# Siyou-Li/u2Tokenizer

Measured on NVIDIA H100. Metric: ct_volumes_per_sec, higher is better.
Workload: dtype bf16

## Files before the change

include/u2b200.h:

```cpp
#ifndef U2B200_H_
#define U2B200_H_

#include <stdint.h>

#if defined(__GNUC__)
#define U2_API __attribute__((visibility("default")))
#else
#define U2_API
#endif

#ifdef __cplusplus
extern "C" {
#endif

#define U2_OK 0
#define U2_ERR_ARG (-1)
#define U2_ERR_CUDA (-2)
#define U2_ERR_UNSUPPORTED (-3)

#define U2_DT_BF16 0
#define U2_DT_F32 1

#define U2_ACT_NONE 0
#define U2_ACT_GELU 1
// ... 97 lines not shown
} u2_rope_desc;
U2_API int u2_rope_bf16(void* x, const u2_rope_desc* desc, void* stream);

U2_API int u2_decode_attention_bf16(const void* q, const void* k_cache, const void* v_cache, void* out,
                                    int32_t B, int32_t Hq, int32_t Hkv, int32_t dh, int32_t Tmax, int32_t T,
                                    const int32_t* T_dev, int64_t ldq, int64_t ldo, float scale, int32_t T_per_seq,
                                    const int32_t* kv_src, int64_t ld_kv_src, void* stream);
U2_API int u2_decode_attention_window_bf16(const void* q, const void* k_cache, const void* v_cache, void* out,
                                           int32_t B, int32_t Hq, int32_t Hkv, int32_t dh, int32_t Tmax, int32_t T,
                                           const int32_t* T_dev, int64_t ldq, int64_t ldo, float scale,
                                           int32_t T_per_seq, const int32_t* kv_src, int64_t ld_kv_src,
                                           int32_t window, void* stream);

typedef struct u2_gemv_desc {
  int32_t B, N, K;
  int64_t ldx, ldw, ldy, ldr;
  int32_t y_dtype;
  const void* residual;
  const float* norm_gamma;
  float norm_eps;
  int32_t silu_pair;
} u2_gemv_desc;
U2_API int u2_gemv_bf16(const void* x, const void* w, void* y, const u2_gemv_desc* desc, void* stream);
U2_API int u2_argmax_f32(const float* logits, int64_t* out, uint64_t* scratch, int32_t B, int32_t V, int64_t ld,
                         void* stream);

#define U2_DLIN_STREAMK128 0
#define U2_DLIN_TILES64 1
typedef struct u2_dlinear_desc {
  int32_t B, N, K;
  int64_t ldx, ldw, ldy, ldr, ldxg;
  int32_t y_dtype;
  float* ws;
  int32_t* counters;
  const float* ssq_in;
  float eps;
  const void* residual;
  int32_t silu_pair;
  const float* gamma_next;
  void* xg;
  float* ssq_out;
  float* ssq_zero;
  int32_t pdl;
  void* dbg;
  int64_t ws_elems;
  const int32_t* dep_flags;
  int32_t dep_shift;
  int32_t* out_flags;
  int32_t sched;
} u2_dlinear_desc;
U2_API int u2_dlinear_bf16(const void* x, const void* w, void* y, const u2_dlinear_desc* desc, void* stream);
U2_API int64_t u2_dlinear_ws_elems(int32_t N, int32_t K);
typedef struct u2_dlinear_next {
  int32_t pre_stages;
  int32_t lookahead_units;
  int32_t n;
  const void* w[2];
  int32_t N[2], K[2];
  int64_t ldw[2];
  int32_t units[2];
} u2_dlinear_next;
U2_API int u2_dlinear_multi_bf16(const void* const* x, const void* const* w, void* const* y,
                                 const u2_dlinear_desc* descs, int32_t n_ops, uint32_t* gridbar,
                                 const int32_t* step_dev, int32_t pdl, const u2_dlinear_next* next, void* stream);
U2_API int u2_decode_embed_bf16(const int64_t* ids, const void* table, const float* gamma, void* x, void* xg,
                                float* ssq, float* ssq_zero, int32_t* step_counter, int32_t B, int32_t E,
                                int64_t vocab, void* stream);

typedef struct u2_fused_decode_desc {
  int32_t B, Hq, Hkv, dh, Tmax, pos;
  const int32_t* pos_dev;
  int64_t ldq, ldo;
  const float* q_norm_w;
  const float* k_norm_w;
  float eps;
  const float* inv_freq;
  float scale;
  int32_t kv_splits;
  int32_t pdl;
  int32_t pos_per_seq;
  const int32_t* kv_src;
  int64_t ld_kv_src;
  int32_t window;
} u2_fused_decode_desc;
U2_API int u2_decode_attention_fused_bf16(const void* qkv, void* k_cache, void* v_cache, void* out,
                                          const u2_fused_decode_desc* desc, void* stream);

U2_API int u2_topk_rows_f32(const float* scores, int64_t* out_idx, int32_t rows, int32_t T, int32_t K, int64_t ld,
                            int64_t idx_offset_per_row, void* stream);

typedef struct u2_fa_desc {
  int32_t B, H, Sq, Sk, dh;
  float scale;
  int64_t q_sb, q_ss, q_sh;
  int64_t k_sb, k_ss, k_sh;
  int64_t v_sb, v_ss, v_sh;
  int64_t out_sb, out_ss;
  float* lse;
} u2_fa_desc;
U2_API int u2_flash_attention_d64_bf16(const void* q, const void* k, const void* v, void* out, const u2_fa_desc* desc,
                                       void* stream);

U2_API int u2_sample_f32(const float* logits, int64_t* out, int32_t B, int32_t V, int64_t ld, float temperature,
                         int32_t top_k, float top_p, uint64_t seed, const int32_t* step_dev, int32_t step,
                         void* stream);

typedef struct u2_sample_params {
  float temperature;
  int32_t top_k;
  float top_p;
  int32_t reserved;
  uint64_t seed;
} u2_sample_params;
U2_API int u2_sample_dev_f32(const float* logits, int64_t* out, int32_t B, int32_t V, int64_t ld,
                             const u2_sample_params* params_dev, const int32_t* step_dev, int32_t step, void* stream);

#define U2_LP_MAX_EOS 8
#define U2_LP_MAX_BAD_WORDS 256
#define U2_LP_MAX_BAD_TOKENS 2048
typedef struct u2_logits_proc_params {
  float penalty;
  float inv_penalty;
  int32_t ngram;
  int32_t min_new;
  int32_t n_eos;
  int32_t n_bad;
  int32_t eos[U2_LP_MAX_EOS];
  int32_t bad_off[U2_LP_MAX_BAD_WORDS + 1];
  int32_t bad_tok[U2_LP_MAX_BAD_TOKENS];
} u2_logits_proc_params;
U2_API int u2_logits_process_f32(float* logits, int32_t B, int32_t V, int64_t ld, const int64_t* ids, int32_t* hist,
                                 int64_t ld_hist, int32_t hist_cap, const u2_logits_proc_params* params_dev,
                                 const int32_t* step_dev, int32_t step, void* stream);

#define U2_BEAM_MAX_BEAMS 16
#define U2_BEAM_MAX_EOS 8
#define U2_BEAM_MAX_KEEP 144
typedef struct u2_beam_params {
  double length_penalty;
  int32_t num_beams;
  int32_t beams_to_keep;
  int32_t early_stopping;
  int32_t max_new_tokens;
  int32_t n_eos;
  int32_t reserved;
  int32_t eos[U2_BEAM_MAX_EOS];
} u2_beam_params;
typedef struct u2_beam_step_desc {
  const u2_beam_params* params;
  int32_t prompts, V;
  const float* cand_val;
  const int32_t* cand_tok;
  float* running;
  float* fin_score;
  int32_t* fin_info;
  int32_t* flags;
  int64_t* ids;
  int32_t* rec;
  int64_t ld_rec;
  int32_t rec_rows;
  int32_t* kv_src;
  int64_t ld_kv_src;
  const int32_t* pos_dev;
  int32_t* hist;
  int64_t ld_hist;
  int32_t hist_cap;
// ... 50 lines not shown
```

u2tokenizer_b200/_lib.py:

```python
from __future__ import annotations

import ctypes as C
from pathlib import Path

_LIB_PATH = Path(__file__).resolve().parent / "libu2b200.so"
_lib = None


class GemmDesc(C.Structure):
    _fields_ = [
        ("M", C.c_int32), ("N", C.c_int32), ("K", C.c_int32),
        ("zi", C.c_int32), ("zo", C.c_int32), ("b_zi_div", C.c_int32),
        ("lda", C.c_int64), ("a_stride_zi", C.c_int64), ("a_stride_zo", C.c_int64),
        ("ldb", C.c_int64), ("b_stride_zi", C.c_int64), ("b_stride_zo", C.c_int64),
        ("ldc", C.c_int64), ("c_stride_zi", C.c_int64), ("c_stride_zo", C.c_int64),
        ("c_dtype", C.c_int32), ("alpha", C.c_float),
        ("bias", C.c_void_p),
        ("act", C.c_int32),
        ("residual", C.c_void_p),
        ("ldr", C.c_int64),
        ("res_row_mod", C.c_int32),
        ("row_div", C.c_int32), ("row_stride", C.c_int32), ("row_off", C.c_int32),
        ("block_n", C.c_int32),
        ("a_mn", C.c_int32), ("b_mn", C.c_int32),
# ... 1 lines not shown
        ("rowvec", C.c_void_p),
        ("rv_stride_zi", C.c_int64), ("rv_stride_zo", C.c_int64),
        ("mul", C.c_void_p),
    ]


class SoftmaxDesc(C.Structure):
    _fields_ = [
        ("in_s0", C.c_int64), ("in_s1", C.c_int64), ("in_s2", C.c_int64),
        ("out_s0", C.c_int64), ("out_s1", C.c_int64), ("out_s2", C.c_int64),
        ("n0", C.c_int32), ("H", C.c_int32), ("S", C.c_int32), ("n", C.c_int32),
        ("scale", C.c_float),
        ("rel_bias", C.c_void_p),
        ("rel_max", C.c_int32),
        ("causal", C.c_int32), ("causal_off", C.c_int32),
        ("zero_pad_to", C.c_int32),
        ("window", C.c_int32),
    ]


class RopeDesc(C.Structure):
    _fields_ = [
        ("rows", C.c_int64), ("ld", C.c_int64),
        ("dh", C.c_int32), ("n_q_heads", C.c_int32), ("n_k_heads", C.c_int32), ("n_v_heads", C.c_int32),
        ("q_norm_w", C.c_void_p), ("k_norm_w", C.c_void_p),
        ("eps", C.c_float),
        ("inv_freq", C.c_void_p),
        ("pos0", C.c_int32), ("pos_div", C.c_int32), ("pos_mod", C.c_int32),
        ("pos0_dev", C.c_void_p),
        ("k_cache", C.c_void_p), ("v_cache", C.c_void_p),
        ("Tmax", C.c_int32), ("rows_per_batch", C.c_int32),
        ("pos0_per_batch", C.c_int32),
    ]


class GemvDesc(C.Structure):
    _fields_ = [
        ("B", C.c_int32), ("N", C.c_int32), ("K", C.c_int32),
        ("ldx", C.c_int64), ("ldw", C.c_int64), ("ldy", C.c_int64), ("ldr", C.c_int64),
        ("y_dtype", C.c_int32),
        ("residual", C.c_void_p),
        ("norm_gamma", C.c_void_p),
        ("norm_eps", C.c_float),
        ("silu_pair", C.c_int32),
    ]


class DlinearDesc(C.Structure):
    _fields_ = [
        ("B", C.c_int32), ("N", C.c_int32), ("K", C.c_int32),
        ("ldx", C.c_int64), ("ldw", C.c_int64), ("ldy", C.c_int64), ("ldr", C.c_int64), ("ldxg", C.c_int64),
        ("y_dtype", C.c_int32),
        ("ws", C.c_void_p), ("counters", C.c_void_p),
        ("ssq_in", C.c_void_p),
        ("eps", C.c_float),
        ("residual", C.c_void_p),
        ("silu_pair", C.c_int32),
        ("gamma_next", C.c_void_p),
        ("xg", C.c_void_p),
        ("ssq_out", C.c_void_p),
        ("ssq_zero", C.c_void_p),
        ("pdl", C.c_int32),
        ("dbg", C.c_void_p),
        ("ws_elems", C.c_int64),
        ("dep_flags", C.c_void_p), ("dep_shift", C.c_int32), ("out_flags", C.c_void_p),
        ("sched", C.c_int32),
    ]


class FusedDecodeDesc(C.Structure):
    _fields_ = [
        ("B", C.c_int32), ("Hq", C.c_int32), ("Hkv", C.c_int32), ("dh", C.c_int32), ("Tmax", C.c_int32),
        ("pos", C.c_int32),
        ("pos_dev", C.c_void_p),
        ("ldq", C.c_int64), ("ldo", C.c_int64),
        ("q_norm_w", C.c_void_p), ("k_norm_w", C.c_void_p),
        ("eps", C.c_float),
        ("inv_freq", C.c_void_p),
        ("scale", C.c_float),
        ("kv_splits", C.c_int32), ("pdl", C.c_int32),
        ("pos_per_seq", C.c_int32),
        ("kv_src", C.c_void_p), ("ld_kv_src", C.c_int64),
        ("window", C.c_int32),
    ]


class DlinearNext(C.Structure):
    _fields_ = [
        ("pre_stages", C.c_int32), ("lookahead_units", C.c_int32), ("n", C.c_int32),
        ("w", C.c_void_p * 2),
        ("N", C.c_int32 * 2), ("K", C.c_int32 * 2),
        ("ldw", C.c_int64 * 2),
        ("units", C.c_int32 * 2),
    ]


class FaDesc(C.Structure):
    _fields_ = [
        ("B", C.c_int32), ("H", C.c_int32), ("Sq", C.c_int32), ("Sk", C.c_int32), ("dh", C.c_int32),
        ("scale", C.c_float),
        ("q_sb", C.c_int64), ("q_ss", C.c_int64), ("q_sh", C.c_int64),
        ("k_sb", C.c_int64), ("k_ss", C.c_int64), ("k_sh", C.c_int64),
        ("v_sb", C.c_int64), ("v_ss", C.c_int64), ("v_sh", C.c_int64),
        ("out_sb", C.c_int64), ("out_ss", C.c_int64),
        ("lse", C.c_void_p),
    ]


class LogprobDesc(C.Structure):
    _fields_ = [
        ("R", C.c_int32), ("V", C.c_int32), ("E", C.c_int32),
        ("ldh", C.c_int64), ("ldw", C.c_int64),
        ("labels", C.c_void_p), ("ws", C.c_void_p), ("ws_bytes", C.c_int64),
        ("lse", C.c_void_p), ("logit_sum", C.c_void_p), ("nll_acc", C.c_void_p),
    ]


class PreprocessInfo(C.Structure):
    _fields_ = [
        ("a_min", C.c_double), ("a_max", C.c_double),
        ("lo", C.c_int32 * 3), ("hi", C.c_int32 * 3), ("out", C.c_int32 * 3),
        ("sigma", C.c_float * 3), ("tail", C.c_int32 * 3), ("status", C.c_int32),
    ]


class PreprocessDesc(C.Structure):
    _fields_ = [
        ("D", C.c_int32), ("H", C.c_int32), ("W", C.c_int32), ("target", C.c_int32), ("pad_depth", C.c_int32),
        ("lower_pct", C.c_double), ("upper_pct", C.c_double),
        ("ws", C.c_void_p), ("ws_bytes", C.c_int64),
    ]


class SoftmaxBwdDesc(C.Structure):
    _fields_ = [
        ("p_s0", C.c_int64), ("p_s1", C.c_int64), ("p_s2", C.c_int64),
        ("dp_s0", C.c_int64), ("dp_s1", C.c_int64), ("dp_s2", C.c_int64),
        ("ds_s0", C.c_int64), ("ds_s1", C.c_int64), ("ds_s2", C.c_int64),
        ("n0", C.c_int32), ("H", C.c_int32), ("S", C.c_int32), ("n", C.c_int32),
        ("zero_pad_to", C.c_int32),
    ]


class AdamWDesc(C.Structure):
    _fields_ = [
        ("lr", C.c_float), ("beta1", C.c_float), ("beta2", C.c_float), ("eps", C.c_float), ("weight_decay", C.c_float),
        ("step", C.c_int32),
        ("grad_scale", C.c_void_p),
        ("seed", C.c_uint64), ("index_offset", C.c_int64),
    ]


class LoraDesc(C.Structure):
    _fields_ = [
        ("M", C.c_int32), ("K", C.c_int32), ("r", C.c_int32), ("n_adapters", C.c_int32),
        ("ldx", C.c_int64), ("ldu", C.c_int64),
        ("scale", C.c_float), ("p", C.c_float),
        ("seed", C.c_uint64),
        ("stream", C.c_int32 * 3),
        ("accumulate", C.c_int32),
    ]


LP_MAX_EOS, LP_MAX_BAD_WORDS, LP_MAX_BAD_TOKENS = 8, 256, 2048


# ... 154 lines not shown
```

u2tokenizer_b200/csrc/attn_small.cu:

```cuda
#include <cooperative_groups.h>
#include <cuda_bf16.h>
#include <math.h>

#include <type_traits>

#include "host_util.h"
#include "u2b200.h"

namespace u2 {

__device__ __forceinline__ float wsum(float v) {
#pragma unroll
  for (int o = 16; o > 0; o >>= 1) v += __shfl_xor_sync(0xffffffffu, v, o);
  return v;
}
__device__ __forceinline__ float wmax(float v) {
#pragma unroll
  for (int o = 16; o > 0; o >>= 1) v = fmaxf(v, __shfl_xor_sync(0xffffffffu, v, o));
  return v;
}

__global__ void __launch_bounds__(128)
temporal_attention_kernel(const __nv_bfloat16* __restrict__ qkv, __nv_bfloat16* __restrict__ out, int C, int N,
                          int H, int dh, long long ld_qkv, long long ld_out, float scale,
// ... 288 lines not shown
  a.k_cache = BF(d->k_cache); a.v_cache = BF(d->v_cache);
  a.Tmax = d->Tmax; a.rows_per_batch = d->rows_per_batch > 0 ? d->rows_per_batch : 1;
  a.pos0_per_batch = d->pos0_per_batch != 0;
  const long long items = d->rows * (long long)(a.n_q_heads + a.n_k_heads + a.n_v_heads);
  rope_kernel<<<(unsigned)((items + 7) / 8), 256, 0, ST(stream)>>>(a);
  U2_CHECK_LAUNCH("rope");
  return U2_OK;
}

static int decode_attention_launch(const void* q, const void* k_cache, const void* v_cache, void* out, int32_t B,
                                   int32_t Hq, int32_t Hkv, int32_t dh, int32_t Tmax, int32_t T, const int32_t* T_dev,
                                   int64_t ldq, int64_t ldo, float scale, int32_t T_per_seq, const int32_t* kv_src,
                                   int64_t ld_kv_src, int32_t window, void* stream) {
  if (!q || !k_cache || !v_cache || !out) return set_error(U2_ERR_ARG, "decode_attention: null pointer");
  if (Hkv <= 0 || Hq % Hkv) return set_error(U2_ERR_ARG, "decode_attention: Hq must be a multiple of Hkv");
  if (!T_dev && (T <= 0 || T > Tmax)) return set_error(U2_ERR_ARG, "decode_attention: need 0 < T <= Tmax");
  if (T_per_seq && !T_dev) return set_error(U2_ERR_ARG, "decode_attention: T_per_seq needs T_dev");
  if (kv_src && ld_kv_src < Tmax) return set_error(U2_ERR_ARG, "decode_attention: kv_src row stride < Tmax");
  if (window < 0) return set_error(U2_ERR_ARG, "decode_attention: window %d < 0", window);
  dim3 grid((unsigned)Hq, (unsigned)B);
#define U2_DA(EPL, IND, WIN, LN) decode_attention_kernel<EPL, IND, WIN, LN><<<grid, 256, 0, ST(stream)>>>(CBF(q), CBF(k_cache), CBF(v_cache), BF(out), Hq, Hkv, Tmax, T, T_dev, ldq, ldo, scale, T_per_seq != 0, kv_src, ld_kv_src, window)
#define U2_DA2(EPL, LN)                                        \
  if (window > 0) {                                            \
    if (kv_src) U2_DA(EPL, true, true, LN);                    \
    else U2_DA(EPL, false, true, LN);                          \
  } else if (kv_src) U2_DA(EPL, true, false, LN);              \
  else U2_DA(EPL, false, false, LN)
  switch (dh) {
    case 32: U2_DA2(1, 32); break;
    case 64: U2_DA2(2, 32); break;
    case 96: U2_DA2(4, 24); break;
    case 128: U2_DA2(4, 32); break;
    default: return set_error(U2_ERR_UNSUPPORTED, "decode_attention: head_dim %d (supported: 32, 64, 96, 128)", dh);
  }
#undef U2_DA2
#undef U2_DA
  U2_CHECK_LAUNCH("decode_attention");
  return U2_OK;
}

extern "C" U2_API int u2_decode_attention_bf16(const void* q, const void* k_cache, const void* v_cache, void* out,
                                               int32_t B, int32_t Hq, int32_t Hkv, int32_t dh, int32_t Tmax,
                                               int32_t T, const int32_t* T_dev, int64_t ldq, int64_t ldo,
                                               float scale, int32_t T_per_seq, const int32_t* kv_src,
                                               int64_t ld_kv_src, void* stream) {
  return decode_attention_launch(q, k_cache, v_cache, out, B, Hq, Hkv, dh, Tmax, T, T_dev, ldq, ldo, scale, T_per_seq,
                                 kv_src, ld_kv_src, 0, stream);
}

extern "C" U2_API int u2_decode_attention_window_bf16(const void* q, const void* k_cache, const void* v_cache,
                                                      void* out, int32_t B, int32_t Hq, int32_t Hkv, int32_t dh,
                                                      int32_t Tmax, int32_t T, const int32_t* T_dev, int64_t ldq,
                                                      int64_t ldo, float scale, int32_t T_per_seq,
                                                      const int32_t* kv_src, int64_t ld_kv_src, int32_t window,
                                                      void* stream) {
  return decode_attention_launch(q, k_cache, v_cache, out, B, Hq, Hkv, dh, Tmax, T, T_dev, ldq, ldo, scale, T_per_seq,
                                 kv_src, ld_kv_src, window, stream);
}

namespace u2 {

constexpr int kFaMaxG = 8;
template <int kDh, int kG>
struct FaCfg {
  static constexpr int kWarps = (kG * kDh * 16 * 4 > 40 * 1024) ? 8 : 16;
};

struct FusedDecodeArgs {
  const __nv_bfloat16* qkv;
  long long ldq;
  __nv_bfloat16* kc;
  __nv_bfloat16* vc;
  __nv_bfloat16* out;
  long long ldo;
  int Hq, Hkv, Tmax;
  const int* pos_dev;
  int pos_per_seq;
  int pos_host;
  const float* q_norm_w;
  const float* k_norm_w;
  float eps;
  const float* inv_freq;
  float scale;
};
struct FusedDecodeIndArgs : FusedDecodeArgs {
  const int* kv_src;
  long long ld_src;
};
struct FusedDecodeWinArgs : FusedDecodeIndArgs {
  int window;
};
template <bool kInd, bool kWin = false>
using FusedArgsT = std::conditional_t<kWin, FusedDecodeWinArgs, std::conditional_t<kInd, FusedDecodeIndArgs, FusedDecodeArgs>>;
template <bool kWin>
__device__ __forceinline__ int window_lo(const FusedArgsT<false, kWin>& a, int pos) {
  if constexpr (kWin) return a.window > 0 ? max(0, pos - a.window + 1) : 0;
  else return 0;
}
template <int kDh>
struct PvMap {
  static constexpr int kEpl = kDh == 96 ? 4 : kDh / 32;
  static constexpr int kLanes = kDh / kEpl;
};
template <bool kInd>
__device__ __forceinline__ long long kv_src_delta(const FusedArgsT<kInd>& a, int b, int t, int pos, long long row_elems) {
  if constexpr (kInd) return kv_src_delta<true>(a.kv_src, a.ld_src, b, t, pos, row_elems);
  else return 0;
}

template <int kDh>
__device__ __forceinline__ void norm_rope_head(const __nv_bfloat16* src, const float* nw, float eps,
                                               const float* inv_freq, int pos, float mul, float* dst_f32,
                                               __nv_bfloat16* dst_bf16, int lane) {
  constexpr int half = kDh / 2;
  float rstd = 1.f;
  if (nw) {
    float ss = 0.f;
    for (int e = lane; e < kDh; e += 32) {
      const float v = __bfloat162float(src[e]);
      ss += v * v;
    }
    ss = wsum(ss);
    rstd = rsqrtf(ss / kDh + eps);
  }
  for (int i = lane; i < half; i += 32) {
    float x1 = __bfloat162float(src[i]), x2 = __bfloat162float(src[i + half]);
    if (nw) {
      x1 = x1 * rstd * nw[i];
      x2 = x2 * rstd * nw[i + half];
    }
    float sn, cs;
    sincosf((float)pos * inv_freq[i], &sn, &cs);
    const __nv_bfloat16 o1 = __float2bfloat16(x1 * cs - x2 * sn);
    const __nv_bfloat16 o2 = __float2bfloat16(x2 * cs + x1 * sn);
    if (dst_bf16) {
      dst_bf16[i] = o1;
      dst_bf16[i + half] = o2;
    }
    if (dst_f32) {
      dst_f32[i] = __bfloat162float(o1) * mul;
      dst_f32[i + half] = __bfloat162float(o2) * mul;
    }
  }
}

template <int kDh, int kG, bool kInd, bool kWin = false>
__global__ void __launch_bounds__(FaCfg<kDh, kG>::kWarps * 32)
fused_decode_attention_kernel(const FusedArgsT<kInd, kWin> a) {
  constexpr int kFaWarps = FaCfg<kDh, kG>::kWarps;
  constexpr int kEpl = PvMap<kDh>::kEpl;
  constexpr int kLanes = PvMap<kDh>::kLanes;
  constexpr int kPf = 16;
  const int hk = blockIdx.x, b = blockIdx.y;
  const int warp = threadIdx.x >> 5, lane = threadIdx.x & 31;
  const int le = kLanes == 32 ? lane : min(lane, kLanes - 1);
  asm volatile("griddepcontrol.wait;" ::: "memory");
  asm volatile("griddepcontrol.launch_dependents;" ::: "memory");
  const int pos = a.pos_dev ? a.pos_dev[a.pos_per_seq ? b : 0] : a.pos_host;
  const int T = min(pos + 1, a.Tmax);
  const int lo = window_lo<kWin>(a, pos);
  __shared__ __align__(16) float s_q[kG][kDh];
  __shared__ float s_m[kFaWarps][kG], s_l[kFaWarps][kG];
  __shared__ float s_acc[kFaWarps][kG][kDh];

  const __nv_bfloat16* row = a.qkv + (long long)b * a.ldq;
  __nv_bfloat16* kbase = a.kc + ((long long)b * a.Hkv + hk) * a.Tmax * kDh;
// ... 44 lines not shown
          for (int j = 0; j < 4; ++j) {
            const float2 f2 = __bfloat1622float2(h2[j]);
            kf[2 * j] = f2.x;
            kf[2 * j + 1] = f2.y;
          }
#pragma unroll
          for (int g = 0; g < kG; ++g) {
            const float4 q0 = *reinterpret_cast<const float4*>(&s_q[g][(c0 + c) * 8]);
            const float4 q1 = *reinterpret_cast<const float4*>(&s_q[g][(c0 + c) * 8 + 4]);
            s[g] += kf[0] * q0.x + kf[1] * q0.y + kf[2] * q0.z + kf[3] * q0.w + kf[4] * q1.x + kf[5] * q1.y +
                    kf[6] * q1.z + kf[7] * q1.w;
          }
        }
      }
    } else {
#pragma unroll
      for (int g = 0; g < kG; ++g) s[g] = -INFINITY;
    }
    float p[kG];
#pragma unroll
    for (int g = 0; g < kG; ++g) {
      const float mx = fmaxf(m[g], wmax(s[g]));
      const float corr = __expf(m[g] - mx);
      p[g] = vis ? __expf(s[g] - mx) : 0.f;
      l[g] = l[g] * corr + wsum(p[g]);
#pragma unroll
      for (int i = 0; i < kEpl; ++i) acc[g][i] *= corr;
      m[g] = mx;
    }
    const int nk = min(32, T - t0);
    for (int j0 = 0; j0 < nk; j0 += kPf) {
      float vv[kPf][kEpl];
#pragma unroll
      for (int jj = 0; jj < kPf; ++jj) {
        const int tj = min(t0 + j0 + jj, T - 1);
        long long dj = 0;
        if constexpr (kInd) dj = __shfl_sync(0xffffffffu, dsrc, tj - t0);
        load_epl<kEpl>(vbase + (long long)tj * kDh + dj + le * kEpl, vv[jj]);
      }
#pragma unroll
      for (int jj = 0; jj < kPf; ++jj) {
#pragma unroll
        for (int g = 0; g < kG; ++g) {
          const float pj = __shfl_sync(0xffffffffu, p[g], (j0 + jj) & 31);
#pragma unroll
          for (int i = 0; i < kEpl; ++i) acc[g][i] += pj * vv[jj][i];
        }
      }
    }
  }
#pragma unroll
  for (int g = 0; g < kG; ++g) {
    if (lane == 0) {
      s_m[warp][g] = m[g];
      s_l[warp][g] = l[g];
    }
    if (kLanes == 32 || lane < kLanes) {
#pragma unroll
      for (int i = 0; i < kEpl; ++i) s_acc[warp][g][lane * kEpl + i] = acc[g][i];
    }
  }
  __syncthreads();
  for (int idx = threadIdx.x; idx < kG * kDh; idx += blockDim.x) {
    const int g = idx / kDh, e = idx - g * kDh;
    float gm = -INFINITY;
#pragma unroll
    for (int w = 0; w < kFaWarps; ++w) gm = fmaxf(gm, s_m[w][g]);
    float gl = 0.f, o = 0.f;
#pragma unroll
    for (int w = 0; w < kFaWarps; ++w) {
      if (s_m[w][g] != -INFINITY) {
        const float f = __expf(s_m[w][g] - gm);
        gl += s_l[w][g] * f;
        o += s_acc[w][g][e] * f;
      }
    }
    a.out[(long long)b * a.ldo + (long long)(hk * kG + g) * kDh + e] = __float2bfloat16(o / gl);
  }
}

template <int kDh, int kG, bool kInd, bool kWin = false>
__global__ void __launch_bounds__(256)
fused_decode_attention_split_kernel(const FusedArgsT<kInd, kWin> a) {
  namespace cg = cooperative_groups;
  cg::cluster_group cluster = cg::this_cluster();
  constexpr int kW = 8;
  constexpr int kEpl = PvMap<kDh>::kEpl;
  constexpr int kLanes = PvMap<kDh>::kLanes;
  constexpr int kVw = (kEpl + 1) / 2;
  const int S = (int)gridDim.z, rank = (int)blockIdx.z;
  const int hk = blockIdx.x, b = blockIdx.y;
  const int warp = threadIdx.x >> 5, lane = threadIdx.x & 31;
  const int le = kLanes == 32 ? lane : min(lane, kLanes - 1);
  asm volatile("griddepcontrol.launch_dependents;" ::: "memory");
  const int pos = a.pos_dev ? a.pos_dev[a.pos_per_seq ? b : 0] : a.pos_host;
  const int T = min(pos + 1, a.Tmax);
  const int lo = window_lo<kWin>(a, pos);
  __shared__ __align__(16) float s_q[kG][kDh];
  __shared__ __align__(16) __nv_bfloat16 s_knew[kDh];
  __shared__ __align__(16) __nv_bfloat16 s_vnew[kDh];
  __shared__ float s_m[kW][kG], s_l[kW][kG];
  __shared__ float s_acc[kW][kG][kDh];
  __shared__ float c_m[kG], c_l[kG];
  __shared__ __align__(16) float c_o[kG][kDh];

  const __nv_bfloat16* row = a.qkv + (long long)b * a.ldq;
  __nv_bfloat16* kbase = a.kc + ((long long)b * a.Hkv + hk) * a.Tmax * kDh;
  __nv_bfloat16* vbase = a.vc + ((long long)b * a.Hkv + hk) * a.Tmax * kDh;

  uint4 ku[kDh / 8];
  uint32_t vw[32][kVw];
  int t0 = (lo & ~31) + (warp * S + rank) * 32;
  const long long row_elems = (long long)a.Hkv * a.Tmax * kDh;
  auto request = [&](int base) {
    const int t = min(base + lane, T - 1);
    const long long dsrc = kv_src_delta<kInd>(a, b, t, pos, row_elems);
    const uint4* kr = reinterpret_cast<const uint4*>(kbase + (long long)t * kDh + dsrc);
#pragma unroll
    for (int c = 0; c < kDh / 8; ++c) ku[c] = kr[c];
#pragma unroll
    for (int jj = 0; jj < 32; ++jj) {
      const int tj = min(base + jj, T - 1);
      long long dj = 0;
      if constexpr (kInd) dj = __shfl_sync(0xffffffffu, dsrc, tj - base);
      const __nv_bfloat16* vp = vbase + (long long)tj * kDh + dj + le * kEpl;
      if constexpr (kEpl == 4) {
        const uint2 u = *reinterpret_cast<const uint2*>(vp);
        vw[jj][0] = u.x;
        vw[jj][1] = u.y;
      } else if constexpr (kEpl == 2) {
        vw[jj][0] = *reinterpret_cast<const uint32_t*>(vp);
      } else {
        vw[jj][0] = *reinterpret_cast<const unsigned short*>(vp);
      }
    }
  };
  if (t0 < T) request(t0);
  asm volatile("griddepcontrol.wait;" ::: "memory");

  for (int job = warp; job < kG + 2; job += kW) {
    if (job == kG) {
      norm_rope_head<kDh>(row + (long long)(a.Hq + hk) * kDh, a.k_norm_w, a.eps, a.inv_freq, pos, 1.f, nullptr, s_knew, lane);
      __syncwarp();
      if (rank == 0)
        for (int e = lane; e < kDh; e += 32) kbase[(long long)pos * kDh + e] = s_knew[e];
    } else if (job == kG + 1) {
      const __nv_bfloat16* v = row + (long long)(a.Hq + a.Hkv + hk) * kDh;
      for (int e = lane; e < kDh; e += 32) {
        const __nv_bfloat16 x = v[e];
        s_vnew[e] = x;
        if (rank == 0) vbase[(long long)pos * kDh + e] = x;
      }
    } else {
      norm_rope_head<kDh>(row + (long long)(hk * kG + job) * kDh, a.q_norm_w, a.eps, a.inv_freq, pos, a.scale, s_q[job],
                          nullptr, lane);
    }
  }
  __syncthreads();

  float m[kG], l[kG], acc[kG][kEpl];
#pragma unroll
  for (int g = 0; g < kG; ++g) {
    m[g] = -INFINITY;
    l[g] = 0.f;
#pragma unroll
    for (int i = 0; i < kEpl; ++i) acc[g][i] = 0.f;
  }
  while (t0 < T) {
    const int t = t0 + lane;
    if (t == pos) {
#pragma unroll
      for (int c = 0; c < kDh / 8; ++c) ku[c] = reinterpret_cast<const uint4*>(s_knew)[c];
    }
    float s[kG];
#pragma unroll
    for (int g = 0; g < kG; ++g) s[g] = 0.f;
#pragma unroll
    for (int c = 0; c < kDh / 8; ++c) {
      const __nv_bfloat162* h2 = reinterpret_cast<const __nv_bfloat162*>(&ku[c]);
      float kf[8];
#pragma unroll
      for (int j = 0; j < 4; ++j) {
        const float2 f2 = __bfloat1622float2(h2[j]);
        kf[2 * j] = f2.x;
        kf[2 * j + 1] = f2.y;
      }
#pragma unroll
      for (int g = 0; g < kG; ++g) {
        const float4 q0 = *reinterpret_cast<const float4*>(&s_q[g][c * 8]);
        const float4 q1 = *reinterpret_cast<const float4*>(&s_q[g][c * 8 + 4]);
        s[g] += kf[0] * q0.x + kf[1] * q0.y + kf[2] * q0.z + kf[3] * q0.w + kf[4] * q1.x + kf[5] * q1.y + kf[6] * q1.z +
                kf[7] * q1.w;
      }
    }
    float p[kG];
    const bool vis = t < T && (!kWin || t >= lo);
#pragma unroll
    for (int g = 0; g < kG; ++g) {
      if (!vis) s[g] = -INFINITY;
      const float mx = fmaxf(m[g], wmax(s[g]));
      const float corr = __expf(m[g] - mx);
      p[g] = vis ? __expf(s[g] - mx) : 0.f;
      l[g] = l[g] * corr + wsum(p[g]);
#pragma unroll
      for (int i = 0; i < kEpl; ++i) acc[g][i] *= corr;
      m[g] = mx;
    }
#pragma unroll
    for (int jj = 0; jj < 32; ++jj) {
      float vf[kEpl];
      if (t0 + jj == pos) {
#pragma unroll
        for (int i = 0; i < kEpl; ++i) vf[i] = __bfloat162float(s_vnew[le * kEpl + i]);
      } else if constexpr (kEpl == 4) {
        const float2 x = __bfloat1622float2(*reinterpret_cast<const __nv_bfloat162*>(&vw[jj][0]));
        const float2 y = __bfloat1622float2(*reinterpret_cast<const __nv_bfloat162*>(&vw[jj][1]));
        vf[0] = x.x; vf[1] = x.y; vf[2] = y.x; vf[3] = y.y;
      } else if constexpr (kEpl == 2) {
        const float2 x = __bfloat1622float2(*reinterpret_cast<const __nv_bfloat162*>(&vw[jj][0]));
        vf[0] = x.x; vf[1] = x.y;
      } else {
        vf[0] = __uint_as_float(vw[jj][0] << 16);
      }
#pragma unroll
      for (int g = 0; g < kG; ++g) {
        const float pj = __shfl_sync(0xffffffffu, p[g], jj);
#pragma unroll
        for (int i = 0; i < kEpl; ++i) acc[g][i] += pj * vf[i];
      }
    }
    t0 += S * kW * 32;
    if (t0 < T) request(t0);
  }
#pragma unroll
  for (int g = 0; g < kG; ++g) {
    if (lane == 0) {
      s_m[warp][g] = m[g];
      s_l[warp][g] = l[g];
    }
    if (kLanes == 32 || lane < kLanes) {
#pragma unroll
      for (int i = 0; i < kEpl; ++i) s_acc[warp][g][lane * kEpl + i] = acc[g][i];
    }
  }
  __syncthreads();
  for (int idx = threadIdx.x; idx < kG * kDh; idx += blockDim.x) {
    const int g = idx / kDh, e = idx - g * kDh;
    float gm = -INFINITY;
#pragma unroll
    for (int w = 0; w < kW; ++w) gm = fmaxf(gm, s_m[w][g]);
    float gl = 0.f, o = 0.f;
#pragma unroll
    for (int w = 0; w < kW; ++w) {
      if (s_m[w][g] != -INFINITY) {
        const float f = __expf(s_m[w][g] - gm);
        gl += s_l[w][g] * f;
        o += s_acc[w][g][e] * f;
      }
    }
    c_o[g][e] = o;
    if (e == 0) {
      c_m[g] = gm;
      c_l[g] = gl;
    }
  }
  cluster.sync();
  if (rank == 0) {
    for (int idx = threadIdx.x; idx < kG * kDh; idx += blockDim.x) {
      const int g = idx / kDh, e = idx - g * kDh;
      float gm = -INFINITY;
      for (int r = 0; r < S; ++r) gm = fmaxf(gm, *cluster.map_shared_rank(&c_m[g], r));
      float gl = 0.f, o = 0.f;
      for (int r = 0; r < S; ++r) {
        const float mr = *cluster.map_shared_rank(&c_m[g], r);
        if (mr != -INFINITY) {
          const float f = __expf(mr - gm);
          gl += *cluster.map_shared_rank(&c_l[g], r) * f;
          o += *cluster.map_shared_rank(&c_o[g][e], r) * f;
        }
      }
      a.out[(long long)b * a.ldo + (long long)(hk * kG + g) * kDh + e] = __float2bfloat16(o / gl);
    }
  }
  cluster.sync();
}

template <int kDh, int kG, bool kInd, bool kWin>
static int launch_fused_decode_split(const FusedArgsT<kInd, kWin>& a, dim3 grid, bool pdl, cudaStream_t st) {
  cudaLaunchConfig_t cfg = {};
  cfg.gridDim = grid;
  cfg.blockDim = dim3(256);
  cfg.dynamicSmemBytes = 0;
  cfg.stream = st;
  cudaLaunchAttribute attr[2];
  attr[0].id = cudaLaunchAttributeClusterDimension;
  attr[0].val.clusterDim.x = 1;
  attr[0].val.clusterDim.y = 1;
  attr[0].val.clusterDim.z = grid.z;
  attr[1].id = cudaLaunchAttributeProgrammaticStreamSerialization;
  attr[1].val.programmaticStreamSerializationAllowed = 1;
  cfg.attrs = attr;
  cfg.numAttrs = pdl ? 2 : 1;
  cudaError_t e = cudaLaunchKernelEx(&cfg, fused_decode_attention_split_kernel<kDh, kG, kInd, kWin>, a);
  if (e != cudaSuccess) return set_error(U2_ERR_CUDA, "decode_attention_fused (split-KV) launch: %s", cudaGetErrorString(e));
  return U2_OK;
}

template <int kDh, bool kInd, bool kWin = false>
static int launch_fused_decode(const FusedArgsT<kInd, kWin>& a, int G, dim3 grid, bool pdl, cudaStream_t st) {
  if (grid.z > 1) {
    switch (G) {
      case 1: return launch_fused_decode_split<kDh, 1, kInd, kWin>(a, grid, pdl, st);
      case 2: return launch_fused_decode_split<kDh, 2, kInd, kWin>(a, grid, pdl, st);
      case 4: return launch_fused_decode_split<kDh, 4, kInd, kWin>(a, grid, pdl, st);
      case 8: return launch_fused_decode_split<kDh, 8, kInd, kWin>(a, grid, pdl, st);
      default: return set_error(U2_ERR_UNSUPPORTED, "decode_attention_fused: Hq/Hkv = %d (supported 1, 2, 4, 8)", G);
    }
  }
  switch (G) {
    case 1: fused_decode_attention_kernel<kDh, 1, kInd, kWin><<<grid, FaCfg<kDh, 1>::kWarps * 32, 0, st>>>(a); break;
    case 2: fused_decode_attention_kernel<kDh, 2, kInd, kWin><<<grid, FaCfg<kDh, 2>::kWarps * 32, 0, st>>>(a); break;
    case 4: fused_decode_attention_kernel<kDh, 4, kInd, kWin><<<grid, FaCfg<kDh, 4>::kWarps * 32, 0, st>>>(a); break;
    case 8: fused_decode_attention_kernel<kDh, 8, kInd, kWin><<<grid, FaCfg<kDh, 8>::kWarps * 32, 0, st>>>(a); break;
    default: return set_error(U2_ERR_UNSUPPORTED, "decode_attention_fused: Hq/Hkv = %d (supported 1, 2, 4, 8)", G);
  }
  return U2_OK;
}

template <int kDh>
static int launch_fused_decode(const FusedDecodeWinArgs& a, int G, dim3 grid, bool pdl, cudaStream_t st) {
  if (a.window > 0) {
    if (a.kv_src) return launch_fused_decode<kDh, true, true>(a, G, grid, pdl, st);
    return launch_fused_decode<kDh, false, true>(a, G, grid, pdl, st);
  }
  if (a.kv_src) return launch_fused_decode<kDh, true>(static_cast<const FusedDecodeIndArgs&>(a), G, grid, pdl, st);
  return launch_fused_decode<kDh, false>(static_cast<const FusedDecodeArgs&>(a), G, grid, pdl, st);
}

}

extern "C" U2_API int u2_decode_attention_fused_bf16(const void* qkv, void* k_cache, void* v_cache, void* out,
                                                     const u2_fused_decode_desc* d, void* stream) {
  using namespace u2;
  if (!qkv || !k_cache || !v_cache || !out || !d || !d->inv_freq) return set_error(U2_ERR_ARG, "decode_attention_fused: null pointer");
  if (d->Hkv <= 0 || d->Hq % d->Hkv || d->Hq / d->Hkv > kFaMaxG)
    return set_error(U2_ERR_UNSUPPORTED, "decode_attention_fused: Hq/Hkv must be an integer <= %d", kFaMaxG);
  if (!d->pos_dev && (d->pos < 0 || d->pos >= d->Tmax)) return set_error(U2_ERR_ARG, "decode_attention_fused: position outside the cache");
  if (d->pos_per_seq && !d->pos_dev) return set_error(U2_ERR_ARG, "decode_attention_fused: pos_per_seq needs pos_dev");
  if (d->window < 0) return set_error(U2_ERR_ARG, "decode_attention_fused: window %d < 0", d->window);
  FusedDecodeWinArgs a;
  a.qkv = CBF(qkv); a.ldq = d->ldq;
  a.kc = BF(k_cache); a.vc = BF(v_cache);
  a.out = BF(out); a.ldo = d->ldo;
  a.Hq = d->Hq; a.Hkv = d->Hkv; a.Tmax = d->Tmax;
  a.pos_dev = d->pos_dev; a.pos_per_seq = d->pos_per_seq != 0; a.pos_host = d->pos;
  a.q_norm_w = d->q_norm_w; a.k_norm_w = d->k_norm_w; a.eps = d->eps;
  a.inv_freq = d->inv_freq; a.scale = d->scale;
  a.kv_src = d->kv_src; a.ld_src = d->ld_kv_src;
  a.window = d->window;
  if (a.kv_src && a.ld_src < d->Tmax) return set_error(U2_ERR_ARG, "decode_attention_fused: kv_src row stride < Tmax");
  const int splits = d->kv_splits > 1 ? d->kv_splits : 1;
  if (splits != 1 && splits != 2 && splits != 4 && splits != 8)
    return set_error(U2_ERR_ARG, "decode_attention_fused: kv_splits must be 0/1, 2, 4 or 8 (portable cluster sizes)");
  dim3 grid((unsigned)d->Hkv, (unsigned)d->B, (unsigned)splits);
  const int G = d->Hq / d->Hkv;
  int rc;
  switch (d->dh) {
    case 32: rc = launch_fused_decode<32>(a, G, grid, d->pdl != 0, ST(stream)); break;
    case 64: rc = launch_fused_decode<64>(a, G, grid, d->pdl != 0, ST(stream)); break;
    case 96: rc = launch_fused_decode<96>(a, G, grid, d->pdl != 0, ST(stream)); break;
    case 128: rc = launch_fused_decode<128>(a, G, grid, d->pdl != 0, ST(stream)); break;
    default: return set_error(U2_ERR_UNSUPPORTED, "decode_attention_fused: head_dim %d (supported 32/64/96/128)", d->dh);
  }
  if (rc) return rc;
  U2_CHECK_LAUNCH("decode_attention_fused");
  return U2_OK;
}
```

u2tokenizer_b200/ops.py:

```python
from __future__ import annotations

import ctypes as C
from typing import Optional

import torch

from . import _lib
from ._lib import GemmDesc

BF16 = torch.bfloat16
F32 = torch.float32

ACT_NONE, ACT_GELU, ACT_SILU = 0, 1, 2
DT_BF16, DT_F32 = 0, 1


def _stream() -> int:
    return torch.cuda.current_stream().cuda_stream


def _ptr(t: Optional[torch.Tensor]) -> Optional[int]:
    return None if t is None else t.data_ptr()


# ... 341 lines not shown
    sc = _argmax_scratch.get(logits.device)
    if sc is None:
        sc = _argmax_scratch[logits.device] = torch.zeros(1024, device=logits.device, dtype=torch.int64)
    _lib.check(_lib.load().u2_argmax_f32(logits.data_ptr(), out.data_ptr(), sc.data_ptr(), B, V, logits.stride(0),
                                         _stream()), "u2_argmax_f32")
    return out


def _dlinear_desc(x, w, out, *, ws, counters, ssq_in=None, eps=1e-6, residual=None, silu_pair=False, gamma_next=None,
                  xg=None, ssq_out=None, ssq_zero=None, pdl=True, dbg=None, sched=0, dep_flags=None, dep_shift=1,
                  out_flags=None):
    _need_cuda(x, w, out, ws, counters, ssq_in, residual, gamma_next, xg, ssq_out, ssq_zero)
    d = _lib.DlinearDesc()
    d.B, d.N, d.K = x.shape[0], w.shape[0], w.shape[1]
    if counters.numel() < (d.N + 63) // 64 + (ssq_out is not None):
        raise ValueError("dlinear counters too small: ceil(N / 64) int32, + 1 with ssq_out")
    d.ws_elems = ws.numel()
    d.ldx, d.ldw, d.ldy = x.stride(0), w.stride(0), out.stride(0)
    d.ldr = residual.stride(0) if residual is not None else 0
    d.ldxg = xg.stride(0) if xg is not None else 0
    d.y_dtype = DT_BF16 if out.dtype == BF16 else DT_F32
    d.ws, d.counters = ws.data_ptr(), counters.data_ptr()
    d.ssq_in = _ptr(ssq_in)
    d.eps = eps
    d.residual = _ptr(residual)
    d.silu_pair = int(silu_pair)
    d.gamma_next = _ptr(gamma_next)
    d.xg = _ptr(xg)
    d.ssq_out = _ptr(ssq_out)
    d.ssq_zero = _ptr(ssq_zero)
    d.pdl = int(pdl)
    d.dbg = _ptr(dbg)
    _need_cuda(dep_flags, out_flags)
    d.dep_flags, d.dep_shift, d.out_flags = _ptr(dep_flags), dep_shift, _ptr(out_flags)
    d.sched = int(sched)
    return d


def dlinear_ws_elems(N: int, K: int) -> int:
    return int(_lib.load().u2_dlinear_ws_elems(N, K))


def dlinear_new_ws(n_elems: int, device="cuda", lead=()) -> torch.Tensor:
    return torch.full((*lead, max(int(n_elems), 4)), -1, device=device, dtype=torch.int32).view(F32)


def dlinear(x: torch.Tensor, w: torch.Tensor, out: torch.Tensor, **kw):
    d = _dlinear_desc(x, w, out, **kw)
    _lib.check(_lib.load().u2_dlinear_bf16(x.data_ptr(), w.data_ptr(), out.data_ptr(), C.byref(d), _stream()),
               "u2_dlinear_bf16")
    return out


def dlinear_multi(ops_list, *, gridbar: torch.Tensor, step_dev: torch.Tensor, pdl: bool = True,
                  lookahead_units: int = 0, next_weights=(), pre_stages: int = 0):
    n = len(ops_list)
    descs = (_lib.DlinearDesc * n)()
    xs, ws_, ys = (C.c_void_p * n)(), (C.c_void_p * n)(), (C.c_void_p * n)()
    for i, (x, w, out, kw) in enumerate(ops_list):
        descs[i] = _dlinear_desc(x, w, out, **kw)
        xs[i], ws_[i], ys[i] = x.data_ptr(), w.data_ptr(), out.data_ptr()
    _need_cuda(gridbar, step_dev)
    nx = _lib.DlinearNext()
    nx.lookahead_units = lookahead_units
    nx.pre_stages = pre_stages
    nx.n = len(next_weights)
    for j, (wn, units) in enumerate(next_weights):
        _need_cuda(wn)
        nx.w[j], nx.N[j], nx.K[j], nx.ldw[j], nx.units[j] = wn.data_ptr(), wn.shape[0], wn.shape[1], wn.stride(0), units
    _lib.check(_lib.load().u2_dlinear_multi_bf16(xs, ws_, ys, descs, n, gridbar.data_ptr(), step_dev.data_ptr(),
                                                 int(pdl), C.byref(nx), _stream()), "u2_dlinear_multi_bf16")


def decode_embed(ids: torch.Tensor, table: torch.Tensor, gamma: torch.Tensor, x: torch.Tensor, xg: torch.Tensor,
                 ssq: torch.Tensor, ssq_zero: Optional[torch.Tensor], step_counter: Optional[torch.Tensor] = None):
    _need_cuda(ids, table, gamma, x, xg, ssq, ssq_zero, step_counter)
    _lib.check(_lib.load().u2_decode_embed_bf16(ids.data_ptr(), table.data_ptr(), gamma.data_ptr(), x.data_ptr(),
                                                xg.data_ptr(), ssq.data_ptr(), _ptr(ssq_zero), _ptr(step_counter),
                                                ids.numel(),
                                                table.shape[1], table.shape[0], _stream()), "u2_decode_embed_bf16")
    return x


def decode_attention_fused(qkv: torch.Tensor, k_cache: torch.Tensor, v_cache: torch.Tensor, out: torch.Tensor, *,
                           B: int, Hq: int, Hkv: int, dh: int, Tmax: int, inv_freq: torch.Tensor, scale: float,
                           pos: int = 0, pos_dev=None, q_norm_w=None, k_norm_w=None, eps: float = 1e-6, kv_splits: int = 1,
                           pdl: bool = False, pos_per_seq: bool = False, kv_src: Optional[torch.Tensor] = None,
                           window: int = 0):
    _need_cuda(qkv, k_cache, v_cache, out, inv_freq, pos_dev, q_norm_w, k_norm_w, kv_src)
    _check_kv_src(kv_src, B, Tmax)
    d = _lib.FusedDecodeDesc()
    d.B, d.Hq, d.Hkv, d.dh, d.Tmax, d.pos = B, Hq, Hkv, dh, Tmax, pos
    d.pos_dev = _ptr(pos_dev)
    d.ldq, d.ldo = qkv.stride(0), out.stride(0)
    d.q_norm_w, d.k_norm_w, d.eps = _ptr(q_norm_w), _ptr(k_norm_w), eps
    d.inv_freq = inv_freq.data_ptr()
    d.scale = scale
    d.kv_splits = int(kv_splits)
    d.pdl = 1 if pdl else 0
    d.pos_per_seq = 1 if pos_per_seq else 0
    d.kv_src = _ptr(kv_src)
    d.ld_kv_src = kv_src.stride(0) if kv_src is not None else 0
    d.window = int(window or 0)
    _lib.check(_lib.load().u2_decode_attention_fused_bf16(qkv.data_ptr(), k_cache.data_ptr(), v_cache.data_ptr(),
                                                          out.data_ptr(), C.byref(d), _stream()),
               "u2_decode_attention_fused_bf16")
    return out


def topk_rows(scores: torch.Tensor, k: int, idx_offset_per_row: int = 0) -> torch.Tensor:
    _need_cuda(scores)
    if scores.dtype != F32 or scores.stride(1) != 1:
        raise TypeError("topk_rows expects fp32 rows")
    rows, T = scores.shape
    out = torch.empty(rows, k, device=scores.device, dtype=torch.int64)
    _lib.check(_lib.load().u2_topk_rows_f32(scores.data_ptr(), out.data_ptr(), rows, T, k, scores.stride(0),
                                            idx_offset_per_row, _stream()), "u2_topk_rows_f32")
    return out


def flash_attention_d64(q: torch.Tensor, k: torch.Tensor, v: torch.Tensor, out: torch.Tensor, scale: float,
                        lse: Optional[torch.Tensor] = None):
    _need_cuda(q, k, v, out)
    B, Sq, H, dh = q.shape
    Sk = k.shape[1]
    if dh != 64 or q.stride(3) != 1 or k.stride(3) != 1 or v.stride(3) != 1 or out.stride(2) != 1 or v.shape != k.shape:
        raise ValueError("flash_attention_d64: head_dim must be 64 with a contiguous last dim, v shaped like k")
    d = _lib.FaDesc()
    d.B, d.H, d.Sq, d.Sk, d.dh, d.scale = B, H, Sq, Sk, dh, scale
    d.q_sb, d.q_ss, d.q_sh = q.stride(0), q.stride(1), q.stride(2)
    d.k_sb, d.k_ss, d.k_sh = k.stride(0), k.stride(1), k.stride(2)
    d.v_sb, d.v_ss, d.v_sh = v.stride(0), v.stride(1), v.stride(2)
    d.out_sb, d.out_ss = out.stride(0), out.stride(1)
    _need_cuda(lse)
    if lse is not None and (lse.dtype != F32 or not lse.is_contiguous() or lse.numel() != B * H * Sq):
        raise ValueError("flash_attention_d64: lse must be contiguous fp32 [B, H, Sq]")
    d.lse = _ptr(lse)
    _lib.check(_lib.load().u2_flash_attention_d64_bf16(q.data_ptr(), k.data_ptr(), v.data_ptr(), out.data_ptr(),
                                                       C.byref(d), _stream()), "u2_flash_attention_d64_bf16")
    return out


def sample(logits: torch.Tensor, out: Optional[torch.Tensor] = None, *, temperature: float = 1.0, top_k: int = 50,
           top_p: float = 1.0, seed: int = 0, step: int = 0, step_dev=None) -> torch.Tensor:
    _need_cuda(logits, step_dev)
    B, V = logits.shape
    if out is None:
        out = torch.empty(B, device=logits.device, dtype=torch.int64)
    _lib.check(_lib.load().u2_sample_f32(logits.data_ptr(), out.data_ptr(), B, V, logits.stride(0), temperature,
                                         int(top_k), float(top_p), int(seed) & ((1 << 64) - 1), _ptr(step_dev),
                                         int(step), _stream()), "u2_sample_f32")
    return out


def sample_params(device, temperature: float, top_k: int, top_p: float, seed: int,
                  out: Optional[torch.Tensor] = None) -> torch.Tensor:
    import struct
    if not temperature > 0:
        raise ValueError("sample: temperature must be > 0")
    if not 0 < top_p <= 1:
        raise ValueError("sample: top_p must be in (0, 1]")
    raw = struct.pack("<fifiQ", float(temperature), int(top_k), float(top_p), 0, int(seed) & ((1 << 64) - 1))
    host = torch.frombuffer(bytearray(raw), dtype=torch.uint8)
    if out is None:
        return host.to(device)
    out.copy_(host)
    return out


def sample_dev(logits: torch.Tensor, params: torch.Tensor, out: Optional[torch.Tensor] = None, *, step: int = 0,
               step_dev=None) -> torch.Tensor:
    _need_cuda(logits, params, step_dev)
    B, V = logits.shape
    if params.dtype != torch.uint8 or params.numel() != 24:
        raise ValueError("sample_dev: params must be the 24-byte block of sample_params()")
    if out is None:
        out = torch.empty(B, device=logits.device, dtype=torch.int64)
    _lib.check(_lib.load().u2_sample_dev_f32(logits.data_ptr(), out.data_ptr(), B, V, logits.stride(0), params.data_ptr(),
                                             _ptr(step_dev), int(step), _stream()), "u2_sample_dev_f32")
    return out


def logits_proc_params(device, vocab_size: int, *, repetition_penalty: float = 1.0, no_repeat_ngram_size: int = 0,
                       min_new_tokens: int = 0, eos_token_ids=(), bad_words_ids=(),
                       out: Optional[torch.Tensor] = None) -> torch.Tensor:
    import numpy as np
# ... 190 lines not shown
```

Measured before the change: 2.173.

## Replace cluster DSMEM split-KV merge with global partials and last-block ticket

The split-KV decode attention kernel no longer launches as a thread-block cluster that merges partial softmax state through distributed shared memory and two cluster syncs. Each split block now writes its max, sum and output partials to a global workspace, increments a per-(batch, kv-head) atomic ticket, and the last arriving block performs the merge and resets the ticket. This drops the cluster launch constraint and the idle waits in cluster.sync. In exchange it adds global memory traffic, fences, an atomic per block, and cached host-side workspace buffers.

```diff
diff --git a/include/u2b200.h b/include/u2b200.h
--- a/include/u2b200.h
+++ b/include/u2b200.h
@@ -203,6 +203,9 @@
   const int32_t* kv_src;
   int64_t ld_kv_src;
   int32_t window;
+  int32_t* split_ticket;
+  float* split_part;
+  int64_t split_ticket_n, split_part_n;
 } u2_fused_decode_desc;
 U2_API int u2_decode_attention_fused_bf16(const void* qkv, void* k_cache, void* v_cache, void* out,
                                           const u2_fused_decode_desc* desc, void* stream);
diff --git a/u2tokenizer_b200/_lib.py b/u2tokenizer_b200/_lib.py
--- a/u2tokenizer_b200/_lib.py
+++ b/u2tokenizer_b200/_lib.py
@@ -107,6 +107,8 @@
         ("pos_per_seq", C.c_int32),
         ("kv_src", C.c_void_p), ("ld_kv_src", C.c_int64),
         ("window", C.c_int32),
+        ("split_ticket", C.c_void_p), ("split_part", C.c_void_p),
+        ("split_ticket_n", C.c_int64), ("split_part_n", C.c_int64),
     ]
 
 
diff --git a/u2tokenizer_b200/csrc/attn_small.cu b/u2tokenizer_b200/csrc/attn_small.cu
--- a/u2tokenizer_b200/csrc/attn_small.cu
+++ b/u2tokenizer_b200/csrc/attn_small.cu
@@ -394,6 +394,8 @@
   float eps;
   const float* inv_freq;
   float scale;
+  int* split_ticket;
+  float* split_part;
 };
 struct FusedDecodeIndArgs : FusedDecodeArgs {
   const int* kv_src;
@@ -604,9 +606,8 @@
 template <int kDh, int kG, bool kInd, bool kWin = false>
 __global__ void __launch_bounds__(256)
 fused_decode_attention_split_kernel(const FusedArgsT<kInd, kWin> a) {
-  namespace cg = cooperative_groups;
-  cg::cluster_group cluster = cg::this_cluster();
   constexpr int kW = 8;
+  constexpr int kMaxS = 8;
   constexpr int kEpl = PvMap<kDh>::kEpl;
   constexpr int kLanes = PvMap<kDh>::kLanes;
   constexpr int kVw = (kEpl + 1) / 2;
@@ -623,8 +624,7 @@
   __shared__ __align__(16) __nv_bfloat16 s_vnew[kDh];
   __shared__ float s_m[kW][kG], s_l[kW][kG];
   __shared__ float s_acc[kW][kG][kDh];
-  __shared__ float c_m[kG], c_l[kG];
-  __shared__ __align__(16) float c_o[kG][kDh];
+  __shared__ int s_last;
 
   const __nv_bfloat16* row = a.qkv + (long long)b * a.ldq;
   __nv_bfloat16* kbase = a.kc + ((long long)b * a.Hkv + hk) * a.Tmax * kDh;
@@ -766,6 +766,9 @@
     }
   }
   __syncthreads();
+  constexpr int kSlot = 2 * kG + kG * kDh;
+  const int pair = b * a.Hkv + hk;
+  float* part = a.split_part + ((long long)pair * S + rank) * kSlot;
   for (int idx = threadIdx.x; idx < kG * kDh; idx += blockDim.x) {
     const int g = idx / kDh, e = idx - g * kDh;
     float gm = -INFINITY;
@@ -780,31 +783,46 @@
         o += s_acc[w][g][e] * f;
       }
     }
-    c_o[g][e] = o;
+    part[2 * kG + idx] = o;
     if (e == 0) {
-      c_m[g] = gm;
-      c_l[g] = gl;
-    }
-  }
-  cluster.sync();
-  if (rank == 0) {
-    for (int idx = threadIdx.x; idx < kG * kDh; idx += blockDim.x) {
-      const int g = idx / kDh, e = idx - g * kDh;
-      float gm = -INFINITY;
-      for (int r = 0; r < S; ++r) gm = fmaxf(gm, *cluster.map_shared_rank(&c_m[g], r));
-      float gl = 0.f, o = 0.f;
-      for (int r = 0; r < S; ++r) {
-        const float mr = *cluster.map_shared_rank(&c_m[g], r);
-        if (mr != -INFINITY) {
-          const float f = __expf(mr - gm);
-          gl += *cluster.map_shared_rank(&c_l[g], r) * f;
-          o += *cluster.map_shared_rank(&c_o[g][e], r) * f;
-        }
-      }
-      a.out[(long long)b * a.ldo + (long long)(hk * kG + g) * kDh + e] = __float2bfloat16(o / gl);
-    }
-  }
-  cluster.sync();
+      part[g] = gm;
+      part[kG + g] = gl;
+    }
+  }
+  __threadfence();
+  __syncthreads();
+  if (threadIdx.x == 0) s_last = atomicAdd(a.split_ticket + pair, 1) == S - 1;
+  __syncthreads();
+  if (!s_last) return;
+  __threadfence();
+  const float* parts = a.split_part + (long long)pair * S * kSlot;
+  for (int idx = threadIdx.x; idx < kG * kDh; idx += blockDim.x) {
+    const int g = idx / kDh, e = idx - g * kDh;
+    float mr[kMaxS], lr[kMaxS], orr[kMaxS];
+#pragma unroll
+    for (int r = 0; r < kMaxS; ++r) {
+      if (r < S) {
+        mr[r] = __ldcg(parts + r * kSlot + g);
+        lr[r] = __ldcg(parts + r * kSlot + kG + g);
+        orr[r] = __ldcg(parts + r * kSlot + 2 * kG + idx);
+      }
+    }
+    float gm = -INFINITY;
+#pragma unroll
+    for (int r = 0; r < kMaxS; ++r)
+      if (r < S) gm = fmaxf(gm, mr[r]);
+    float gl = 0.f, o = 0.f;
+#pragma unroll
+    for (int r = 0; r < kMaxS; ++r) {
+      if (r < S && mr[r] != -INFINITY) {
+        const float f = __expf(mr[r] - gm);
+        gl += lr[r] * f;
+        o += orr[r] * f;
+      }
+    }
+    a.out[(long long)b * a.ldo + (long long)(hk * kG + g) * kDh + e] = __float2bfloat16(o / gl);
+  }
+  if (threadIdx.x == 0) a.split_ticket[pair] = 0;
 }
 
 template <int kDh, int kG, bool kInd, bool kWin>
@@ -814,15 +832,11 @@
   cfg.blockDim = dim3(256);
   cfg.dynamicSmemBytes = 0;
   cfg.stream = st;
-  cudaLaunchAttribute attr[2];
-  attr[0].id = cudaLaunchAttributeClusterDimension;
-  attr[0].val.clusterDim.x = 1;
-  attr[0].val.clusterDim.y = 1;
-  attr[0].val.clusterDim.z = grid.z;
-  attr[1].id = cudaLaunchAttributeProgrammaticStreamSerialization;
-  attr[1].val.programmaticStreamSerializationAllowed = 1;
+  cudaLaunchAttribute attr[1];
+  attr[0].id = cudaLaunchAttributeProgrammaticStreamSerialization;
+  attr[0].val.programmaticStreamSerializationAllowed = 1;
   cfg.attrs = attr;
-  cfg.numAttrs = pdl ? 2 : 1;
+  cfg.numAttrs = pdl ? 1 : 0;
   cudaError_t e = cudaLaunchKernelEx(&cfg, fused_decode_attention_split_kernel<kDh, kG, kInd, kWin>, a);
   if (e != cudaSuccess) return set_error(U2_ERR_CUDA, "decode_attention_fused (split-KV) launch: %s", cudaGetErrorString(e));
   return U2_OK;
@@ -880,10 +894,21 @@
   a.inv_freq = d->inv_freq; a.scale = d->scale;
   a.kv_src = d->kv_src; a.ld_src = d->ld_kv_src;
   a.window = d->window;
+  a.split_ticket = nullptr;
+  a.split_part = nullptr;
   if (a.kv_src && a.ld_src < d->Tmax) return set_error(U2_ERR_ARG, "decode_attention_fused: kv_src row stride < Tmax");
   const int splits = d->kv_splits > 1 ? d->kv_splits : 1;
   if (splits != 1 && splits != 2 && splits != 4 && splits != 8)
-    return set_error(U2_ERR_ARG, "decode_attention_fused: kv_splits must be 0/1, 2, 4 or 8 (portable cluster sizes)");
+    return set_error(U2_ERR_ARG, "decode_attention_fused: kv_splits must be 0/1, 2, 4 or 8");
+  if (splits > 1) {
+    const long long pairs = (long long)d->B * d->Hkv;
+    const long long need = pairs * splits * (2 + d->dh) * (long long)(d->Hq / d->Hkv);
+    if (!d->split_ticket || !d->split_part || d->split_ticket_n < pairs || d->split_part_n < need)
+      return set_error(U2_ERR_ARG, "decode_attention_fused: kv_splits %d needs %lld tickets and %lld partial floats",
+                       splits, pairs, need);
+    a.split_ticket = d->split_ticket;
+    a.split_part = d->split_part;
+  }
   dim3 grid((unsigned)d->Hkv, (unsigned)d->B, (unsigned)splits);
   const int G = d->Hq / d->Hkv;
   int rc;
diff --git a/u2tokenizer_b200/ops.py b/u2tokenizer_b200/ops.py
--- a/u2tokenizer_b200/ops.py
+++ b/u2tokenizer_b200/ops.py
@@ -447,6 +447,16 @@
     return x
 
 
+_split_ws_bufs = {}
+
+
+def _split_ws(device: torch.device, dtype: torch.dtype, n: int) -> torch.Tensor:
+    bufs = _split_ws_bufs.setdefault((device, _stream(), dtype), [])
+    if not bufs or bufs[-1].numel() < n:
+        bufs.append(torch.zeros(max(n, 1 << 12), device=device, dtype=dtype))
+    return bufs[-1]
+
+
 def decode_attention_fused(qkv: torch.Tensor, k_cache: torch.Tensor, v_cache: torch.Tensor, out: torch.Tensor, *,
                            B: int, Hq: int, Hkv: int, dh: int, Tmax: int, inv_freq: torch.Tensor, scale: float,
                            pos: int = 0, pos_dev=None, q_norm_w=None, k_norm_w=None, eps: float = 1e-6, kv_splits: int = 1,
@@ -467,6 +477,11 @@
     d.kv_src = _ptr(kv_src)
     d.ld_kv_src = kv_src.stride(0) if kv_src is not None else 0
     d.window = int(window or 0)
+    if kv_splits > 1:
+        tickets = _split_ws(qkv.device, torch.int32, B * Hkv)
+        part = _split_ws(qkv.device, F32, B * Hkv * kv_splits * (2 + dh) * (Hq // Hkv))
+        d.split_ticket, d.split_part = tickets.data_ptr(), part.data_ptr()
+        d.split_ticket_n, d.split_part_n = tickets.numel(), part.numel()
     _lib.check(_lib.load().u2_decode_attention_fused_bf16(qkv.data_ptr(), k_cache.data_ptr(), v_cache.data_ptr(),
                                                           out.data_ptr(), C.byref(d), _stream()),
                "u2_decode_attention_fused_bf16")
```

New measurement: 2.270 (median of 6 runs). +4.5%, better.
